# bittremieux/ANN-SoLo

Measured on AMD Instinct MI355X. Metric: query spectra/sec + recall@k vs brute-force, open-mod search on MassIVE-KB, higher is better.
Workload: dtype f32; 1 GPU; configs[2]: MassIVE-KB-scale synthetic library (2100000 spectra, one charge-2 partition), ivfpq m=32 nlist=4096 nprobe=128 k=1024, open +-500 Da, shifted dot, fragment tol 0.02 Da; library_size=2100000, batch_per_gpu=32768, reference_default_batch_size=16384, global_batch=32768, index=ivfpq, nlist=4096, nprobe=128, k=1024, parallelism=single

## Files before the change

ann_solo_amd/csrc/pq_scan_v3.hip:

```cpp
#include "common.hpp"
#include "hist_topk.hpp"
#include "ivf_kernels.hpp"
#include "pq_tile.hpp"

namespace asl {

constexpr int V3_CHUNK = 256;
constexpr int V3_DEPTH = 1;
constexpr int V3_NT = 0;
constexpr int V3_AHEAD = 8;
constexpr uint32_t V3_MM_DEAD = 0xfffffff0u;
constexpr int V3_WAVES_PER_SIMD = 6;

template <int NT_>
__device__ __forceinline__ uint4 load_codes16(const uint8_t *p) {
  if (NT_) {
    const uint32_t *w = reinterpret_cast<const uint32_t *>(p);
    typedef uint32_t u32x4 __attribute__((ext_vector_type(4)));
    const u32x4 v = __builtin_nontemporal_load(reinterpret_cast<const u32x4 *>(w));
    return make_uint4(v.x, v.y, v.z, v.w);
  }
  return *reinterpret_cast<const uint4 *>(p);
}

struct TileEnt8 {
  uint32_t tile_nv;
  float coarse;
};

struct TileEnt12 {
  uint32_t tile_nv;
  float coarse;
  uint32_t first;
};
constexpr int V3_CHUNK_RANGED = 168;
static_assert(V3_CHUNK_RANGED * sizeof(TileEnt12) <= V3_CHUNK * sizeof(TileEnt8), "the ranged table fits the 2 KB");

template <int CAP, int T, int NW, int DEPTH, bool WIDE, bool RANGED = false, bool SEL = false, bool MM = false>
__global__ __launch_bounds__(64 * NW, (NW == 8 ? (CAP <= 2048 ? V3_WAVES_PER_SIMD : 4) : (CAP <= 2048 ? 3 : 1))) void pq_scan_v3_kernel(
    const float *__restrict__ xq, int d, const float *__restrict__ codebooks, int dsub,
    const float *__restrict__ coarse_D, const int32_t *__restrict__ coarse_I, int nprobe,
    const int32_t *__restrict__ list_offsets, const int32_t *__restrict__ tile_offsets,
    const uint8_t *__restrict__ codes_tiled, const int32_t *__restrict__ ids_tiled, int k,
    float *__restrict__ D, int64_t *__restrict__ I64, int32_t *__restrict__ I32, int set_mode,
    const uint2 *__restrict__ ent, const int32_t *__restrict__ ent_cnt, const int *__restrict__ gate,
    const ScanPostFilter pf, const ScanRanges rg, const unsigned long long *__restrict__ sel, const uint32_t mm_plane) {
  static_assert(!SEL || CAP <= 2048, "the selector is built into the 2048-key instantiations only");
  static_assert(!MM || (!RANGED && !SEL), "the sub-quantiser-major copy exists of the default layout only");
  if (gate && (int)blockIdx.x >= *gate) return;
  static_assert(DEPTH >= 1 && DEPTH <= 3, "rounds of prefetch");
  static_assert(T == 1, "one tile per wave at a time (two lost on registers: profiles/HISTORY.md)");
  constexpr int NT = 64 * NW, ROUND_VECS = NW * 64;
  using TopK = HistTopK<CAP, ROUND_VECS, NT>;
  using Ent = typename std::conditional<RANGED, TileEnt12, TileEnt8>::type;
  extern __shared__ __attribute__((aligned(16))) char smem[];
  float *s_lut = reinterpret_cast<float *>(smem + TopK::lds_bytes());
  Ent *table = reinterpret_cast<Ent *>(s_lut + PQT_KSUB * PQT_M);
  float *s_q = reinterpret_cast<float *>(smem);

  const int tid = threadIdx.x, lane = tid & 63, wave = tid >> 6, q = blockIdx.x;
  constexpr int PP = WIDE ? 2 : 1;
  int my_len[PP], my_tile0[PP], my_nt[PP], my_pre[PP];
  int my_first[PP];
  float my_coarse[PP];
#pragma unroll
  for (int pp = 0; pp < PP; ++pp) {
    my_len[pp] = 0, my_tile0[pp] = 0, my_nt[pp] = 0, my_coarse[pp] = 0.0f, my_first[pp] = 0;
    const int p = tid + pp * NT;
    if (p < nprobe) {
      const int l = coarse_I[(size_t)q * nprobe + p];
      if (l >= 0) {
        if constexpr (RANGED) {
          const int2 r = rg.range[(size_t)q * nprobe + p];
          my_first[pp] = r.x & 63;
          my_len[pp] = r.y > r.x ? r.y - (r.x & ~63) : 0;
          my_tile0[pp] = tile_offsets[l] + (r.x >> 6);
        } else {
          my_len[pp] = list_offsets[l + 1] - list_offsets[l];
          my_tile0[pp] = tile_offsets[l];
        }
        my_nt[pp] = (my_len[pp] + 63) >> 6;
        my_coarse[pp] = coarse_D[(size_t)q * nprobe + p];
      }
    }
  }
  build_lut_cbt<NT>(xq + (size_t)q * d, d, codebooks, dsub, s_q, s_lut, reinterpret_cast<uint8_t *>(table),
                    tid, ent ? ent + (size_t)q * 64 : nullptr,
                    ent ? (xq ? ent_cnt[q] : max(ent_cnt[q], 0)) : -1);

  uint32_t live_u = 0;
  if constexpr (MM) {
    const uint8_t *s_nz = reinterpret_cast<const uint8_t *>(table);
    const int K = reinterpret_cast<const int *>(s_nz)[0];
    uint32_t mine = 0;
    for (int i = tid & 63; i < K; i += 64) mine |= 1u << (s_nz[8 + i] & 31);
#pragma unroll
    for (int o = 32; o > 0; o >>= 1) mine |= (uint32_t)__shfl_xor((int)mine, o);
    live_u = (uint32_t)__builtin_amdgcn_readfirstlane((int)mine);
    __syncthreads();
  }

  int total = 0;
  int *scan_part = reinterpret_cast<int *>(table);
#pragma unroll
  for (int pp = 0; pp < PP; ++pp) {
    int part_total;
    my_pre[pp] = total + block_excl_scan<NW>(my_nt[pp], scan_part, tid, part_total);
    total += part_total;
    __syncthreads();
  }
  total = __builtin_amdgcn_readfirstlane(total);

  TopK top;
  top.init(smem, k, ids_tiled, tid);
  top.out_keys = set_mode == 2 && I64 != nullptr;

  const char *lut_bytes = reinterpret_cast<const char *>(s_lut);
  const int wave_u = __builtin_amdgcn_readfirstlane(wave);
  const int rho = lane >> 4, j = lane & 15;
  const int ma = (rho & 1) ? j + 16 : j, mb = ma ^ 16;
  const uint32_t offA = (uint32_t)ma * 4u, offB = (uint32_t)mb * 4u;
  const bool liveA = (live_u >> ma) & 1u, liveB = (live_u >> mb) & 1u;
  const uint32_t chunkA = MM ? (liveA ? (uint32_t)ma * mm_plane + (uint32_t)(rho * 16) : V3_MM_DEAD) : (uint32_t)(rho * 512 + ma * 16);
  const uint32_t chunkB = liveB ? (uint32_t)mb * mm_plane + (uint32_t)(rho * 16) : V3_MM_DEAD;

  int *s_flag = top.ctl + TopK::C_USER;
  int *s_done = top.ctl + TopK::C_USER + 1;
  if (tid == 0) {
    *s_flag = 0;
    *s_done = 0;
  }
  auto flag_up = [&]() -> int { return __hip_atomic_load(s_flag, __ATOMIC_RELAXED, __HIP_MEMORY_SCOPE_WORKGROUP); };
  auto flag_set = [&](int v) { __hip_atomic_store(s_flag, v, __ATOMIC_RELAXED, __HIP_MEMORY_SCOPE_WORKGROUP); };
  float thr_u = -INFINITY;
  uint32_t thr_hi_u = 0;
  int flag_u = 0;

  constexpr int CHUNK = RANGED ? V3_CHUNK_RANGED : V3_CHUNK;
  for (int c0 = 0; c0 < total; c0 += CHUNK) {
#pragma unroll
    for (int pp = 0; pp < PP; ++pp) {
      asm volatile("" : "+v"(my_pre[pp]), "+v"(my_nt[pp]), "+v"(my_tile0[pp]), "+v"(my_len[pp]));
      const int lo = max(my_pre[pp], c0), hi = min(my_pre[pp] + my_nt[pp], c0 + CHUNK);
      for (int t = lo; t < hi; ++t) {
        const int local = t - my_pre[pp];
        Ent e;
        e.tile_nv = (uint32_t)(my_tile0[pp] + local) | ((uint32_t)(min(64, my_len[pp] - local * 64) - 1) << 26);
        e.coarse = my_coarse[pp];
        if constexpr (RANGED) e.first = local == 0 ? (uint32_t)my_first[pp] : 0u;
        table[t - c0] = e;
      }
    }
    __syncthreads();
    const int nent = min(CHUNK, total - c0);
    constexpr int NS = DEPTH + 1;
    uint4 A[NS], B[NS];
    if constexpr (MM) {
#pragma unroll
      for (int s = 0; s < NS; ++s) A[s] = B[s] = make_uint4(0u, 0u, 0u, 0u);
    }
    struct Tile {
      uint32_t tile_nv;
      float coarse;
      uint32_t first;
      unsigned long long sel;
    } e[NS];
    auto fetch = [&](int i, uint4 &a, uint4 &b, Tile &en, bool real = true) {
      const Ent t = table[i];
      en.tile_nv = __builtin_amdgcn_readfirstlane(t.tile_nv);
      en.coarse = __builtin_bit_cast(float, __builtin_amdgcn_readfirstlane(__builtin_bit_cast(int, t.coarse)));
      if constexpr (RANGED) en.first = __builtin_amdgcn_readfirstlane(t.first);
      if constexpr (SEL) en.sel = sel[en.tile_nv & 0x3ffffffu];
      if constexpr (MM) {
        const uint32_t toff = (en.tile_nv & 0x3ffffffu) * 64u;
        const uint8_t *base = codes_tiled + (size_t)toff;
        uint32_t offa = chunkA, offb = chunkB;
        asm volatile("" : "+v"(offa), "+v"(offb));
        const __amdgpu_buffer_rsrc_t rs = __builtin_amdgcn_make_buffer_rsrc(
            const_cast<uint8_t *>(base), 0, (int)(real ? (uint32_t)PQT_M * mm_plane - toff : 0u), 0x00020000);
        typedef uint32_t u32x4 __attribute__((ext_vector_type(4)));
        const u32x4 va = __builtin_amdgcn_raw_buffer_load_b128(rs, (int)offa, 0, V3_NT ? 2 : 0);
        const u32x4 vb = __builtin_amdgcn_raw_buffer_load_b128(rs, (int)offb, 0, V3_NT ? 2 : 0);
        a = make_uint4(va.x, va.y, va.z, va.w);
        b = make_uint4(vb.x, vb.y, vb.z, vb.w);
      } else {
        const uint8_t *base = codes_tiled + (size_t)(en.tile_nv & 0x3ffffffu) * 2048;
        uint32_t offa = chunkA;
        asm volatile("" : "+v"(offa));
        const uint32_t offb = offa ^ 256u;
        a = load_codes16<V3_NT>(base + offa);
        b = load_codes16<V3_NT>(base + offb);
      }
    };
    float p_score = 0.0f;
    uint32_t p_tile_nv = 0, p_first = 0;
    unsigned long long p_sel = 0;
    bool pending = false;
    auto append = [&]() {
      const int end = (int)(p_tile_nv >> 26);
      bool in = RANGED ? (lane <= end && lane >= (int)p_first) : lane <= end;
      if constexpr (SEL) in = in && ((p_sel >> lane) & 1ull) != 0;
      bool p;
      if (thr_hi_u != 0) {
        float sc = p_score;
        asm volatile("; exact flushes" : "+v"(sc));
        p = in && f2ord(sc) >= thr_hi_u;
      } else {
        p = in && p_score >= thr_u;
      }
      const unsigned long long m = __ballot(p);
      int base = -2;
      if (m) base = top.free_reserve(__popcll(m));
      pending = base == -1;
      if (base >= 0) top.free_write(p, m, p_score, (p_tile_nv << 6) + (uint32_t)lane, base, false);
    };
    auto step = [&](int i, int s) {
      const int fl = flag_up();
      if constexpr (MM)
        fetch(min(i + DEPTH * NW, nent - 1), A[(s + DEPTH) % NS], B[(s + DEPTH) % NS], e[(s + DEPTH) % NS],
              i + DEPTH * NW < nent);
      else if (i + DEPTH * NW < nent)
        fetch(i + DEPTH * NW, A[(s + DEPTH) % NS], B[(s + DEPTH) % NS], e[(s + DEPTH) % NS]);
      flag_u = __builtin_amdgcn_readfirstlane(fl);
      p_score = e[s].coarse + tile_adc<V3_AHEAD>(lut_bytes, A[s], B[s], offA, offB);
      p_tile_nv = e[s].tile_nv;
      if constexpr (RANGED) p_first = e[s].first;
      if constexpr (SEL) p_sel = e[s].sel;
      append();
    };
    int i = wave_u;
#pragma unroll
    for (int s = 0; s < DEPTH; ++s)
      if (i + s * NW < nent) fetch(i + s * NW, A[s], B[s], e[s]);
    bool finished = false;
    for (;;) {
      bool meet = false;
      while (i < nent && !meet) {
#pragma unroll
        for (int s = 0; s < NS; ++s) {
          if (i < nent && !meet) {
            step(i, s);
            i += NW;
            if (pending || flag_u) {
              meet = true;
              if (s + 1 < NS) {
#pragma unroll
                for (int u = 0; u < DEPTH; ++u) {
                  A[u] = A[(s + 1 + u) % NS];
                  B[u] = B[(s + 1 + u) % NS];
                  e[u] = e[(s + 1 + u) % NS];
                }
              }
            }
          }
        }
      }
      if (!meet) {
        if (!finished) {
          if (lane == 0) atomicAdd(s_done, 1);
          finished = true;
        }
        for (;;) {
          flag_u = __builtin_amdgcn_readfirstlane(flag_up());
          if (flag_u ||
              __builtin_amdgcn_readfirstlane(__hip_atomic_load(s_done, __ATOMIC_RELAXED, __HIP_MEMORY_SCOPE_WORKGROUP)) >=
                  NW * (c0 / CHUNK + 1))
            break;
          __builtin_amdgcn_s_sleep(4);
        }
        if (!flag_u) break;
      }
      do {
        if (lane == 0) flag_set(1);
        __syncthreads();
        if (tid == 0) flag_set(0);
        asm volatile("" : "+v"(top.tid));
        top.free_sync(true);
        thr_u = __builtin_bit_cast(float, __builtin_amdgcn_readfirstlane(__builtin_bit_cast(int, top.thr_f)));
        thr_hi_u = (uint32_t)__builtin_amdgcn_readfirstlane((int)top.thr_hi);
        flag_u = 0;
        if (pending) append();
      } while (pending);
    }
    __syncthreads();
  }
  top.free_done(true);
  if constexpr (RANGED) {
    if (set_mode) {
      const int n = top.finish_set(D ? D + (size_t)q * k : nullptr, I64 ? I64 + (size_t)q * k : nullptr,
                                   I32 ? I32 + (size_t)q * k : nullptr, reinterpret_cast<u64 *>(s_lut));
      if (rg.row_len && tid == 0) rg.row_len[q] = n;
    } else {
      top.finish(D ? D + (size_t)q * k : nullptr, I64 ? I64 + (size_t)q * k : nullptr,
                 I32 ? I32 + (size_t)q * k : nullptr);
    }
  } else if (set_mode && CAP * 9 <= PQT_KSUB * PQT_M * 4)
    top.finish_set(D ? D + (size_t)q * k : nullptr, I64 ? I64 + (size_t)q * k : nullptr,
                   I32 ? I32 + (size_t)q * k : nullptr, reinterpret_cast<u64 *>(s_lut), &pf, q);
  else if (set_mode && CAP * 8 <= PQT_KSUB * PQT_M * 4)
    top.finish_set(D ? D + (size_t)q * k : nullptr, I64 ? I64 + (size_t)q * k : nullptr,
                   I32 ? I32 + (size_t)q * k : nullptr, reinterpret_cast<u64 *>(s_lut));
  else
    top.finish(D ? D + (size_t)q * k : nullptr, I64 ? I64 + (size_t)q * k : nullptr,
               I32 ? I32 + (size_t)q * k : nullptr);
}

template <int CAP, int T, int NW, int DEPTH, bool WIDE, bool RANGED = false, bool SEL = false, bool MM = false>
static int launch_v3(const float *xq, int nq, int d, const float *codebooks, int dsub,
                     const float *coarse_D, const int32_t *coarse_I, int nprobe,
                     const int32_t *list_offsets, const int32_t *tile_offsets,
                     const uint8_t *codes_tiled, const int32_t *ids_tiled, int k, float *D,
                     int64_t *I64, int32_t *I32, int set_mode, const uint2 *ent,
                     const int32_t *ent_cnt, const int *gate, const ScanPostFilter &pf,
                     const ScanRanges &rg, const unsigned long long *sel = nullptr, uint32_t mm_plane = 0) {
  constexpr size_t TABLE = RANGED ? V3_CHUNK_RANGED * sizeof(TileEnt12) : V3_CHUNK * sizeof(TileEnt8);
  if ((size_t)d * 4 > (size_t)CAP * 8 || dsub > 64 || (size_t)d * 2 + 8 > TABLE || d != PQT_M * dsub)
    return fail(ASL_ERR_CAPACITY, "pq scan: d=%d too large for the LDS staging", d);
  const size_t lds = HistTopK<CAP, NW * T * 64, 64 * NW>::lds_bytes() + (size_t)PQT_KSUB * PQT_M * 4 +
                     (size_t)V3_CHUNK * sizeof(TileEnt8);
  if (lds > 160 * 1024) return fail(ASL_ERR_CAPACITY, "pq scan: k=%d does not fit LDS", k);
  if (lds > 64 * 1024)
    HIP_TRY(hipFuncSetAttribute((const void *)pq_scan_v3_kernel<CAP, T, NW, DEPTH, WIDE, RANGED, SEL, MM>,
                                hipFuncAttributeMaxDynamicSharedMemorySize, (int)lds));
  hipLaunchKernelGGL((pq_scan_v3_kernel<CAP, T, NW, DEPTH, WIDE, RANGED, SEL, MM>), dim3(nq), dim3(64 * NW), lds, stream(),
                     xq, d, codebooks, dsub, coarse_D, coarse_I, nprobe, list_offsets, tile_offsets,
                     codes_tiled, ids_tiled, k, D, I64, I32, set_mode, ent, ent_cnt, gate, pf, rg, sel, mm_plane);
  ASL_CHECK_LAUNCH();
  return ASL_OK;
}

bool pq_scan_tiled_supported(int m, int ksub, int k, int nprobe) {
  return m == PQT_M && ksub == PQT_KSUB && nprobe <= 1024 && k >= 1 && k <= TK_MAX_K;
}

int pq_scan_v3(const float *xq, int nq, int d, const float *codebooks, int dsub,
               const float *coarse_D, const int32_t *coarse_I, int nprobe,
               const int32_t *list_offsets, const int32_t *tile_offsets,
               const uint8_t *codes_tiled, const int32_t *ids_tiled, int k, float *D,
               int64_t *I64, int32_t *I32, int set_mode, const uint2 *ent, const int32_t *ent_cnt,
               const int *gate, const ScanPostFilter *post, const ScanRanges *ranges,
               const unsigned long long *sel, const uint8_t *codes_mm, uint32_t mm_plane) {
  if (nq <= 0) return ASL_OK;
  ScanPostFilter pf;
  if (post && post->idpay) {
    if (!(set_mode == 1 && I32 && k + 256 + 512 <= 2048))
      return fail(ASL_ERR_STATE, "pq scan: a post-filter needs set-mode int32 rows and k <= 1280");
    pf = *post;
  }
  const ScanRanges none;
#define V3_ARGS xq, nq, d, codebooks, dsub, coarse_D, coarse_I, nprobe, list_offsets, tile_offsets, \
                codes_tiled, ids_tiled, k, D, I64, I32, set_mode, ent, ent_cnt, gate, pf
  if (sel && (set_mode == 2 || k + 256 + 512 > 2048))
    return fail(ASL_ERR_STATE, "pq scan: a selector needs k <= 1280 and rows of ids");
  if (ranges && ranges->range) {
    if (pf.idpay || set_mode == 2 || k + 256 + 512 > 2048)
      return fail(ASL_ERR_STATE, "pq scan: the window scan needs k <= 1280, rows of ids and no post-filter");
    if (sel) {
      if (nprobe > 512) return launch_v3<2048, 1, 8, V3_DEPTH, true, true, true>(V3_ARGS, *ranges, sel);
      return launch_v3<2048, 1, 8, V3_DEPTH, false, true, true>(V3_ARGS, *ranges, sel);
    }
    if (nprobe > 512) return launch_v3<2048, 1, 8, V3_DEPTH, true, true>(V3_ARGS, *ranges);
    return launch_v3<2048, 1, 8, V3_DEPTH, false, true>(V3_ARGS, *ranges);
  }
  if (sel) {
    if (nprobe > 512) return launch_v3<2048, 1, 8, V3_DEPTH, true, false, true>(V3_ARGS, none, sel);
    return launch_v3<2048, 1, 8, V3_DEPTH, false, false, true>(V3_ARGS, none, sel);
  }
  if (codes_mm && !gate) {
#define V3_MM_ARGS xq, nq, d, codebooks, dsub, coarse_D, coarse_I, nprobe, list_offsets, tile_offsets, \
                   codes_mm, ids_tiled, k, D, I64, I32, set_mode, ent, ent_cnt, gate, pf, none, nullptr, mm_plane
    if (nprobe > 512) {
      if (k + 256 + 512 <= 2048) return launch_v3<2048, 1, 8, V3_DEPTH, true, false, false, true>(V3_MM_ARGS);
      return launch_v3<4096, 1, 8, V3_DEPTH, true, false, false, true>(V3_MM_ARGS);
    }
    if (k + 256 + 512 <= 2048) return launch_v3<2048, 1, 8, V3_DEPTH, false, false, false, true>(V3_MM_ARGS);
    return launch_v3<4096, 1, 8, V3_DEPTH, false, false, false, true>(V3_MM_ARGS);
#undef V3_MM_ARGS
  }
  if (nprobe > 512) {
    if (k + 256 + 512 <= 2048) return launch_v3<2048, 1, 8, V3_DEPTH, true>(V3_ARGS, none);
    return launch_v3<4096, 1, 8, V3_DEPTH, true>(V3_ARGS, none);
  }
  if (k + 256 + 512 <= 2048) return launch_v3<2048, 1, 8, V3_DEPTH, false>(V3_ARGS, none);
  return launch_v3<4096, 1, 8, V3_DEPTH, false>(V3_ARGS, none);
#undef V3_ARGS
}

__global__ void window_ranges_kernel(const double *__restrict__ q_pmz, int nq,
                                     const int32_t *__restrict__ coarse_I, int nprobe,
                                     const int32_t *__restrict__ list_offsets,
                                     const int32_t *__restrict__ tile_offsets,
                                     const float *__restrict__ wkey, int charge, double tol, int mode,
                                     int2 *__restrict__ ranges, unsigned long long *__restrict__ acc) {
  const int64_t i = block_linear() * blockDim.x + threadIdx.x;
  unsigned long long cnt = 0;
  if (i < (int64_t)nq * nprobe) {
    const int l = coarse_I[i];
    int2 r = make_int2(0, 0);
    if (l >= 0) {
      const float *key = wkey + (size_t)tile_offsets[l] * 64;
      const int n = list_offsets[l + 1] - list_offsets[l];
      const QueryWindow w = query_window(q_pmz, i / nprobe, mode);
      const double qm = w.q;
      int a = 0, b = n;
      while (a < b) {
        const int mid = (a + b) >> 1;
        if ((double)key[mid] < qm) a = mid + 1; else b = mid;
      }
      const int p0 = a;
      a = mode == ASL_TOL_INTERVAL ? p0 : 0, b = p0;
      while (a < b) {
        const int mid = (a + b) >> 1;
        if (precursor_ok(qm, key[mid], charge, tol, mode)) b = mid; else a = mid + 1;
      }
      const int lo = a;
      a = p0, b = (mode == ASL_TOL_INTERVAL && !(w.q <= w.hi)) ? p0 : n;
      while (a < b) {
        const int mid = (a + b) >> 1;
        if (precursor_ok(w, key[mid], charge, tol, mode)) a = mid + 1; else b = mid;
      }
      r = make_int2(lo, a);
      cnt = (unsigned long long)(a - lo);
    }
    ranges[i] = r;
  }
  if (acc) {
    for (int off = 32; off > 0; off >>= 1) cnt += __shfl_xor(cnt, off);
    if ((threadIdx.x & 63) == 0 && cnt) atomicAdd(acc, cnt);
  }
}

int window_ranges(const double *q_pmz, int nq, const int32_t *coarse_I, int nprobe,
                  const int32_t *list_offsets, const int32_t *tile_offsets, const float *wkey, int charge,
                  double tol, int mode, int2 *ranges, unsigned long long *acc) {
  const int64_t n = (int64_t)nq * nprobe;
  if (n <= 0) return ASL_OK;
  hipLaunchKernelGGL(window_ranges_kernel, grid_2d(cdiv(n, 256)), dim3(256), 0, stream(), q_pmz, nq, coarse_I,
                     nprobe, list_offsets, tile_offsets, wkey, charge, tol, mode, ranges, acc);
  ASL_CHECK_LAUNCH();
  return ASL_OK;
}

__global__ void tile_codes_kernel(const uint8_t *__restrict__ codes, const int32_t *__restrict__ ids,
                                  const int32_t *__restrict__ dst_slot, int64_t n,
                                  uint8_t *__restrict__ codes_tiled,
                                  int32_t *__restrict__ ids_tiled) {
  const int64_t t = block_linear() * blockDim.x + threadIdx.x;
  if (t >= n * PQT_M) return;
  const int64_t i = t >> 5;
  const int m = (int)(t & 31);
  const int32_t slot = dst_slot[i];
  const int64_t tile = slot >> 6;
  const int v = slot & 63, rho = v >> 4, b = (v & 15) ^ (m & 15);
  codes_tiled[tile * 2048 + rho * 512 + m * 16 + b] = codes[t];
  if (m == 0) ids_tiled[tile * 64 + v] = ids[i];
}

int tile_codes(const uint8_t *codes, const int32_t *ids, const int32_t *dst_slot, int64_t n,
               int64_t ntiles, uint8_t *codes_tiled, int32_t *ids_tiled) {
  HIP_TRY(hipMemsetAsync(codes_tiled, 0, (size_t)ntiles * 2048, stream()));
  HIP_TRY(hipMemsetAsync(ids_tiled, 0xff, (size_t)ntiles * 64 * 4, stream()));
  if (n <= 0) return ASL_OK;
  hipLaunchKernelGGL(tile_codes_kernel, grid_2d(cdiv(n * PQT_M, 256)), dim3(256), 0,
                     stream(), codes, ids, dst_slot, n, codes_tiled, ids_tiled);
  ASL_CHECK_LAUNCH();
  return ASL_OK;
}

__global__ void mmajor_codes_kernel(const uint4 *__restrict__ codes_tiled, int64_t ntiles, uint32_t plane,
                                    uint8_t *__restrict__ codes_mm) {
  const int64_t t = block_linear() * blockDim.x + threadIdx.x;
  if (t >= ntiles * 128) return;
  const int64_t tile = t >> 7;
  const int rho = (int)(t >> 5) & 3, m = (int)(t & 31);
  *reinterpret_cast<uint4 *>(codes_mm + (size_t)m * plane + (size_t)tile * 64 + rho * 16) = codes_tiled[t];
}

int mmajor_codes(const uint8_t *codes_tiled, int64_t ntiles, uint32_t plane, uint8_t *codes_mm) {
  HIP_TRY(hipMemsetAsync(codes_mm, 0, (size_t)plane * PQT_M, stream()));
  if (ntiles <= 0) return ASL_OK;
  hipLaunchKernelGGL(mmajor_codes_kernel, grid_2d(cdiv(ntiles * 128, 256)), dim3(256), 0, stream(),
                     reinterpret_cast<const uint4 *>(codes_tiled), ntiles, plane, codes_mm);
  ASL_CHECK_LAUNCH();
  return ASL_OK;
}

__global__ __launch_bounds__(256) void tile_selector_kernel(const int32_t *__restrict__ slot_ids, int64_t ntiles,
                                                            const uint8_t *__restrict__ keep, int64_t n,
                                                            unsigned long long *__restrict__ words) {
  const int64_t tile = block_linear() * 4 + (threadIdx.x >> 6);
  const int lane = threadIdx.x & 63;
  if (tile >= ntiles) return;
  const int32_t id = slot_ids[tile * 64 + lane];
  const unsigned long long m = __ballot(id >= 0 && id < n && keep[id] != 0);
  if (lane == 0) words[tile] = m;
}

int tile_selector(const int32_t *slot_ids, int64_t ntiles, const uint8_t *keep, int64_t n,
                  unsigned long long *words) {
  if (ntiles <= 0) return ASL_OK;
  hipLaunchKernelGGL(tile_selector_kernel, grid_2d(cdiv(ntiles, 4)), dim3(256), 0, stream(), slot_ids, ntiles,
                     keep, n, words);
  ASL_CHECK_LAUNCH();
  return ASL_OK;
}

}
```

Measured before the change: 2.890 million query spectra/s.

## Restructure PQ scan hot loop with ballot-first fast path and LDS address stepping

Splits the per-wave scan loop into a tight hot loop that computes a ballot of threshold passers and only drops into the append and merge path when something passes or a flag is raised. Table entries are now fetched by an incrementing LDS byte address instead of re-indexing. The in-range lane mask is built with scalar bit operations, and the ranged first-lane offset is packed into the top bits of my_tile0 to save registers. Adds disabled padding helpers (zero pad) for instruction-timing experiments. The intent is to cut VALU and SALU work and register pressure per tile, at the cost of more complex resume logic after an early exit.

```diff
diff --git a/ann_solo_amd/csrc/pq_scan_v3.hip b/ann_solo_amd/csrc/pq_scan_v3.hip
--- a/ann_solo_amd/csrc/pq_scan_v3.hip
+++ b/ann_solo_amd/csrc/pq_scan_v3.hip
@@ -10,6 +10,26 @@
 constexpr int V3_NT = 0;
 constexpr int V3_AHEAD = 8;
 constexpr uint32_t V3_MM_DEAD = 0xfffffff0u;
+constexpr int V3_PAD_SALU = 0;
+constexpr int V3_PAD_VALU = 0;
+#define V3_PAD4(op) op " %0, 0\n\t" op " %1, 1\n\t" op " %2, 2\n\t" op " %3, 3\n\t"
+#define V3_PAD16(op) V3_PAD4(op) V3_PAD4(op) V3_PAD4(op) V3_PAD4(op)
+template <int NS_, int NV_>
+__device__ __forceinline__ void v3_pad() {
+  static_assert(NS_ % 16 == 0 && NV_ % 16 == 0, "the padding comes in blocks of 16 instructions");
+#pragma unroll
+  for (int n = 0; n < NS_ / 16; ++n) {
+    uint32_t a, b, c, d;
+    asm volatile(V3_PAD16("s_mov_b32") : "=s"(a), "=s"(b), "=s"(c), "=s"(d));
+  }
+#pragma unroll
+  for (int n = 0; n < NV_ / 16; ++n) {
+    uint32_t a, b, c, d;
+    asm volatile(V3_PAD16("v_mov_b32") : "=v"(a), "=v"(b), "=v"(c), "=v"(d));
+  }
+}
+#undef V3_PAD16
+#undef V3_PAD4
 constexpr int V3_WAVES_PER_SIMD = 6;
 
 template <int NT_>
@@ -61,20 +81,18 @@
   const int tid = threadIdx.x, lane = tid & 63, wave = tid >> 6, q = blockIdx.x;
   constexpr int PP = WIDE ? 2 : 1;
   int my_len[PP], my_tile0[PP], my_nt[PP], my_pre[PP];
-  int my_first[PP];
   float my_coarse[PP];
 #pragma unroll
   for (int pp = 0; pp < PP; ++pp) {
-    my_len[pp] = 0, my_tile0[pp] = 0, my_nt[pp] = 0, my_coarse[pp] = 0.0f, my_first[pp] = 0;
+    my_len[pp] = 0, my_tile0[pp] = 0, my_nt[pp] = 0, my_coarse[pp] = 0.0f;
     const int p = tid + pp * NT;
     if (p < nprobe) {
       const int l = coarse_I[(size_t)q * nprobe + p];
       if (l >= 0) {
         if constexpr (RANGED) {
           const int2 r = rg.range[(size_t)q * nprobe + p];
-          my_first[pp] = r.x & 63;
           my_len[pp] = r.y > r.x ? r.y - (r.x & ~63) : 0;
-          my_tile0[pp] = tile_offsets[l] + (r.x >> 6);
+          my_tile0[pp] = (int)((uint32_t)(tile_offsets[l] + (r.x >> 6)) | ((uint32_t)(r.x & 63) << 26));
         } else {
           my_len[pp] = list_offsets[l + 1] - list_offsets[l];
           my_tile0[pp] = tile_offsets[l];
@@ -140,14 +158,15 @@
   for (int c0 = 0; c0 < total; c0 += CHUNK) {
 #pragma unroll
     for (int pp = 0; pp < PP; ++pp) {
-      asm volatile("" : "+v"(my_pre[pp]), "+v"(my_nt[pp]), "+v"(my_tile0[pp]), "+v"(my_len[pp]));
-      const int lo = max(my_pre[pp], c0), hi = min(my_pre[pp] + my_nt[pp], c0 + CHUNK);
+      asm volatile("" : "+v"(my_pre[pp]), "+v"(my_tile0[pp]), "+v"(my_len[pp]));
+      const int lo = max(my_pre[pp], c0), hi = min(my_pre[pp] + ((my_len[pp] + 63) >> 6), c0 + CHUNK);
       for (int t = lo; t < hi; ++t) {
         const int local = t - my_pre[pp];
         Ent e;
-        e.tile_nv = (uint32_t)(my_tile0[pp] + local) | ((uint32_t)(min(64, my_len[pp] - local * 64) - 1) << 26);
+        const uint32_t tile0 = RANGED ? (uint32_t)my_tile0[pp] & 0x3ffffffu : (uint32_t)my_tile0[pp];
+        e.tile_nv = (tile0 + (uint32_t)local) | ((uint32_t)(min(64, my_len[pp] - local * 64) - 1) << 26);
         e.coarse = my_coarse[pp];
-        if constexpr (RANGED) e.first = local == 0 ? (uint32_t)my_first[pp] : 0u;
+        if constexpr (RANGED) e.first = local == 0 ? (uint32_t)my_tile0[pp] >> 26 : 0u;
         table[t - c0] = e;
       }
     }
@@ -165,22 +184,22 @@
       uint32_t first;
       unsigned long long sel;
     } e[NS];
-    auto fetch = [&](int i, uint4 &a, uint4 &b, Tile &en, bool real = true) {
-      const Ent t = table[i];
-      en.tile_nv = __builtin_amdgcn_readfirstlane(t.tile_nv);
-      en.coarse = __builtin_bit_cast(float, __builtin_amdgcn_readfirstlane(__builtin_bit_cast(int, t.coarse)));
-      if constexpr (RANGED) en.first = __builtin_amdgcn_readfirstlane(t.first);
+    auto fetch = [&](uint32_t taddr, uint4 &a, uint4 &b, Tile &en, uint32_t num_records = 0) {
+      typedef uint32_t u32x2 __attribute__((ext_vector_type(2)));
+      const u32x2 t = *(const __attribute__((address_space(3))) u32x2 *)(uintptr_t)taddr;
+      en.tile_nv = __builtin_amdgcn_readfirstlane(t.x);
+      en.coarse = __builtin_bit_cast(float, __builtin_amdgcn_readfirstlane((int)t.y));
+      if constexpr (RANGED)
+        en.first = __builtin_amdgcn_readfirstlane(*(const __attribute__((address_space(3))) uint32_t *)(uintptr_t)(taddr + 8u));
       if constexpr (SEL) en.sel = sel[en.tile_nv & 0x3ffffffu];
       if constexpr (MM) {
         const uint32_t toff = (en.tile_nv & 0x3ffffffu) * 64u;
         const uint8_t *base = codes_tiled + (size_t)toff;
-        uint32_t offa = chunkA, offb = chunkB;
-        asm volatile("" : "+v"(offa), "+v"(offb));
-        const __amdgpu_buffer_rsrc_t rs = __builtin_amdgcn_make_buffer_rsrc(
-            const_cast<uint8_t *>(base), 0, (int)(real ? (uint32_t)PQT_M * mm_plane - toff : 0u), 0x00020000);
+        const __amdgpu_buffer_rsrc_t rs =
+            __builtin_amdgcn_make_buffer_rsrc(const_cast<uint8_t *>(base), 0, (int)num_records, 0x00020000);
         typedef uint32_t u32x4 __attribute__((ext_vector_type(4)));
-        const u32x4 va = __builtin_amdgcn_raw_buffer_load_b128(rs, (int)offa, 0, V3_NT ? 2 : 0);
-        const u32x4 vb = __builtin_amdgcn_raw_buffer_load_b128(rs, (int)offb, 0, V3_NT ? 2 : 0);
+        const u32x4 va = __builtin_amdgcn_raw_buffer_load_b128(rs, (int)chunkA, 0, V3_NT ? 2 : 0);
+        const u32x4 vb = __builtin_amdgcn_raw_buffer_load_b128(rs, (int)chunkB, 0, V3_NT ? 2 : 0);
         a = make_uint4(va.x, va.y, va.z, va.w);
         b = make_uint4(vb.x, vb.y, vb.z, vb.w);
       } else {
@@ -192,69 +211,104 @@
         b = load_codes16<V3_NT>(base + offb);
       }
     };
+    constexpr uint32_t ENT_STRIDE = NW * sizeof(Ent);
+    const uint32_t mm_size = (uint32_t)PQT_M * mm_plane;
     float p_score = 0.0f;
     uint32_t p_tile_nv = 0, p_first = 0;
     unsigned long long p_sel = 0;
     bool pending = false;
-    auto append = [&]() {
-      const int end = (int)(p_tile_nv >> 26);
-      bool in = RANGED ? (lane <= end && lane >= (int)p_first) : lane <= end;
-      if constexpr (SEL) in = in && ((p_sel >> lane) & 1ull) != 0;
-      bool p;
-      if (thr_hi_u != 0) {
+    auto in_mask = [&]() -> unsigned long long {
+      unsigned long long in = ~0ull >> (~(p_tile_nv >> 26) & 63u);
+      if constexpr (RANGED) in &= ~0ull << (p_first & 63u);
+      if constexpr (SEL) in &= p_sel;
+      return in;
+    };
+    auto passers = [&]() -> unsigned long long { return __ballot(p_score >= thr_u) & in_mask(); };
+    auto append = [&](unsigned long long m, bool thresholded = false) {
+      if (!thresholded && thr_hi_u != 0) {
         float sc = p_score;
         asm volatile("; exact flushes" : "+v"(sc));
-        p = in && f2ord(sc) >= thr_hi_u;
-      } else {
-        p = in && p_score >= thr_u;
-      }
-      const unsigned long long m = __ballot(p);
-      int base = -2;
-      if (m) base = top.free_reserve(__popcll(m));
-      pending = base == -1;
-      if (base >= 0) top.free_write(p, m, p_score, (p_tile_nv << 6) + (uint32_t)lane, base, false);
+        m = __ballot(f2ord(sc) >= thr_hi_u) & in_mask();
+      }
+      pending = false;
+      if (m) {
+        const int base = top.free_reserve(__builtin_amdgcn_readfirstlane(__popcll(m)));
+        pending = base < 0;
+        if (!pending) top.free_write(__builtin_amdgcn_inverse_ballot_w64(m), m, p_score, (p_tile_nv << 6) + (uint32_t)lane, base, false);
+      }
     };
-    auto step = [&](int i, int s) {
+    const uint32_t table_lds = (uint32_t)(uintptr_t)(const __attribute__((address_space(3))) char *)reinterpret_cast<const char *>(table);
+    int i = wave_u;
+    if (i < nent) {
+      uint32_t t0 = table_lds + (uint32_t)i * (uint32_t)sizeof(Ent);
+      asm volatile("" : "+v"(t0));
+#pragma unroll
+      for (int s = 0; s < DEPTH; ++s)
+        if (i + s * NW < nent) fetch(t0 + s * ENT_STRIDE, A[s], B[s], e[s], mm_size);
+    }
+    uint32_t taddr = 0;
+    auto step = [&](int s) {
+      const int f = (s + DEPTH) % NS;
       const int fl = flag_up();
-      if constexpr (MM)
-        fetch(min(i + DEPTH * NW, nent - 1), A[(s + DEPTH) % NS], B[(s + DEPTH) % NS], e[(s + DEPTH) % NS],
-              i + DEPTH * NW < nent);
-      else if (i + DEPTH * NW < nent)
-        fetch(i + DEPTH * NW, A[(s + DEPTH) % NS], B[(s + DEPTH) % NS], e[(s + DEPTH) % NS]);
+      const bool real = i + DEPTH * NW < nent;
+      if constexpr (MM) {
+        taddr += real ? ENT_STRIDE : 0u;
+        fetch(taddr, A[f], B[f], e[f], real ? mm_size : 0u);
+      } else if (real) {
+        taddr += ENT_STRIDE;
+        fetch(taddr, A[f], B[f], e[f]);
+      }
       flag_u = __builtin_amdgcn_readfirstlane(fl);
       p_score = e[s].coarse + tile_adc<V3_AHEAD>(lut_bytes, A[s], B[s], offA, offB);
       p_tile_nv = e[s].tile_nv;
       if constexpr (RANGED) p_first = e[s].first;
       if constexpr (SEL) p_sel = e[s].sel;
-      append();
+      i += NW;
     };
-    int i = wave_u;
-#pragma unroll
-    for (int s = 0; s < DEPTH; ++s)
-      if (i + s * NW < nent) fetch(i + s * NW, A[s], B[s], e[s]);
+    auto hot = [&]() -> int {
+      for (;;) {
+#pragma unroll
+        for (int s = 0; s < NS; ++s) {
+          if (i >= nent) return -1;
+          step(s);
+          v3_pad<V3_PAD_SALU, V3_PAD_VALU>();
+          const unsigned long long m = passers();
+          if (__builtin_expect(((uint32_t)m | (uint32_t)(m >> 32) | (uint32_t)flag_u | thr_hi_u) != 0u, 0)) {
+            if (((uint32_t)flag_u | thr_hi_u) != 0u) return s;
+            append(m, true);
+            if (pending) return s + NS;
+          }
+        }
+      }
+    };
     bool finished = false;
     for (;;) {
+      taddr = table_lds + (uint32_t)(DEPTH == 1 ? min(i, CHUNK - 1) : min(i + (DEPTH - 1) * NW, nent - 1)) * (uint32_t)sizeof(Ent);
+      asm volatile("" : "+v"(taddr));
+      int ev = hot();
+      asm volatile("" : "+s"(ev));
       bool meet = false;
-      while (i < nent && !meet) {
-#pragma unroll
-        for (int s = 0; s < NS; ++s) {
-          if (i < nent && !meet) {
-            step(i, s);
-            i += NW;
-            if (pending || flag_u) {
-              meet = true;
-              if (s + 1 < NS) {
-#pragma unroll
-                for (int u = 0; u < DEPTH; ++u) {
-                  A[u] = A[(s + 1 + u) % NS];
-                  B[u] = B[(s + 1 + u) % NS];
-                  e[u] = e[(s + 1 + u) % NS];
-                }
-              }
+#pragma unroll
+      for (int s = 0; s < NS; ++s) {
+        if (ev < 0 || s < ev % NS || meet) continue;
+        if (s > ev % NS) {
+          if (i >= nent) continue;
+          step(s);
+        }
+        if (!(ev >= NS && s == ev % NS)) append(passers());
+        if (pending || flag_u) {
+          meet = true;
+          if (s + 1 < NS) {
+#pragma unroll
+            for (int u = 0; u < DEPTH; ++u) {
+              A[u] = A[(s + 1 + u) % NS];
+              B[u] = B[(s + 1 + u) % NS];
+              e[u] = e[(s + 1 + u) % NS];
             }
           }
         }
       }
+      if (ev >= 0 && !meet) continue;
       if (!meet) {
         if (!finished) {
           if (lane == 0) atomicAdd(s_done, 1);
@@ -279,7 +333,7 @@
         thr_u = __builtin_bit_cast(float, __builtin_amdgcn_readfirstlane(__builtin_bit_cast(int, top.thr_f)));
         thr_hi_u = (uint32_t)__builtin_amdgcn_readfirstlane((int)top.thr_hi);
         flag_u = 0;
-        if (pending) append();
+        if (pending) append(passers());
       } while (pending);
     }
     __syncthreads();
```

Measured after the change: 2.934 million query spectra/s, median of 6. +1.5%, better.
